# ShenhanQian/SpeechDrivesTemplates

Measured on AMD Instinct MI355X. Metric: training clips/sec (64-frame, 137-kpt) voice2pose_sdt_bp, higher is better.
Workload: dtype f32 (Conv2d forward / input gradient: each fp32 operand split exactly into three bf16 numbers, six bf16 MFMA products per fp32 product, fp32 accumulation -- products exact to 2^-23; everything else fp32 arithmetic)

## Files before the change

__graft_entry__.py:

```python
import os
import subprocess
import sys

REPO = os.path.dirname(os.path.abspath(__file__))
CSRC = os.path.join(REPO, "speechdrivestemplates_amd", "csrc")
LIBDIR = os.path.join(REPO, "speechdrivestemplates_amd", "lib")
LIB = os.path.join(LIBDIR, "libsdt_hip.so")
SOURCES = ["conv.hip", "convsk.hip", "convbf.hip", "norm.hip", "misc.hip", "l0.hip", "chain1d.hip", "render.hip", "speaker_stats.hip",
           "code_pca.hip", "code_axes.hip", "code_clusters.hip", "fgd.hip", "jpeg.hip", "gif.hip", "clip_builder.hip", "optim_guard.hip",
           "tensor_hist.hip", "reg_loss.hip", "bone_loss.hip", "clip_metrics.hip", "long_demo.hip", "sync_metrics.hip", "augment.hip", "speech_gate.hip",
           "pose_augment.hip", "motion_dist.hip", "code_fit.hip"]
HIPCC = os.environ.get("HIPCC", "/opt/rocm/bin/hipcc")
FLAGS = ["--offload-arch=gfx950", "-O3", "-std=c++17", "-fPIC", "-munsafe-fp-atomics", "-Wno-unused-result", "-Wno-unused-value"]


def _stale(out, deps):
    if not os.path.exists(out):
        return True
    t = os.path.getmtime(out)
    return any(os.path.getmtime(d) > t for d in deps)


TUNING_LIB = os.path.join(LIBDIR, "libsdt_hip_tuning.so")


def _headers():
# ... 111 lines not shown
```

include/sdt_hip.h:

```cpp
#ifndef SDT_HIP_H
#define SDT_HIP_H

#include <stdint.h>

#ifdef __cplusplus
extern "C" {
#endif

#define SDT_MAX_TAPS 20

enum sdt_status { SDT_OK = 0, SDT_ERR_ARG = -1, SDT_ERR_LAUNCH = -2, SDT_ERR_UNSUPPORTED = -3 };
enum sdt_dtype { SDT_F32 = 0, SDT_BF16 = 1 };

const char* sdt_last_error(void);
int sdt_abi_version(void);

typedef struct sdt_conv_geom {
    int32_t B, Hi, Wi, Cin;
    int32_t Ho, Wo;
    int32_t Hy, Wy, Cout;
    int32_t sy, sx;
    int32_t osy, osx, ooy, oox;
    int32_t ntaps, Tw;
    int32_t dy[SDT_MAX_TAPS], dx[SDT_MAX_TAPS], wt[SDT_MAX_TAPS];
// ... 54 lines not shown
int64_t sdt_convsk_dw_plan_bytes_t(const sdt_conv_geom* g, int dtype);
int sdt_convsk_dw_plan_build_t(const sdt_conv_geom* g, int dtype, void* out, int64_t out_bytes);
int sdt_convsk_dw_bf16(const void* x, const void* dy, float* dw, const void* plan_host, const void* plan_dev, void* workspace,
                       int64_t xbytes, int64_t ybytes, void* stream);
int sdt_conv_dw_f32(const float* x, const float* dy, float* dw, const sdt_conv_geom* g, void* stream);
int64_t sdt_conv_dw_workspace_bytes(const sdt_conv_geom* g);
int sdt_conv_dw_det_f32(const float* x, const float* dy, float* dw, const sdt_conv_geom* g, void* workspace, int64_t workspace_bytes,
                        void* stream);
int sdt_conv_taps_variant(const sdt_conv_geom* g);
int sdt_conv1d_small_used(const sdt_conv_geom* geoms, int ncls, int splitk);
int sdt_conv_dw_variant(const sdt_conv_geom* g);
int sdt_weight_transpose_f32(const float* w, float* wt, int cout, int taps, int cin, void* stream);
enum { SDT_MATH_F32 = 0, SDT_MATH_BF16 = 1, SDT_MATH_BF16X3 = 3, SDT_MATH_BF16X6 = 6 };
int sdt_set_conv_math(int mode);
int sdt_get_conv_math(void);


int64_t sdt_conv_dw_group_plan_bytes(int n);
int sdt_conv_dw_group_plan(const sdt_conv_geom* const* geoms, int n, void* plan_out, int64_t* workspace_bytes);
int sdt_conv_dw_group_f32(const void* const* x, const void* const* dy, void* const* dw, int n, const void* plan_host, const void* plan_dev,
                          void* workspace, void* stream);
typedef struct sdt_wt_desc {
    const float* w;
    float* wt;
    void* w16;
    void* wt16;
    int32_t cout, taps, cin, tile_begin;
    int32_t planes;
    int32_t reserved;
} sdt_wt_desc;
// ... 21 lines not shown

int sdt_l0_block_fwd_f32(const float* mel, const float* w, float* z, double* mom, float* mean, float* rstd,
                         const float* gamma, const float* beta, float* running_mean, float* running_var,
                         int64_t* num_batches_tracked, int B, int H, int W, int groups, float eps, float momentum,
                         float slope, void* stream);
int sdt_l0_block_bwd_f32(const float* dz, const float* mel, const float* w, const float* mean, const float* rstd,
                         const float* gamma, const float* beta, const double* mom, double* sums, float* dw, float* dgamma,
                         float* dbeta, int B, int H, int W, int groups, float slope, void* stream);
int sdt_l0_block_fwd_t(const float* mel, const float* w, void* z, int z_dtype, double* mom, float* mean, float* rstd,
                       const float* gamma, const float* beta, float* running_mean, float* running_var,
                       int64_t* num_batches_tracked, int B, int H, int W, int groups, float eps, float momentum,
                       float slope, void* stream);
int sdt_l0_block_bwd_t(const void* dz, int dz_dtype, const float* mel, const float* w, const float* mean, const float* rstd,
                       const float* gamma, const float* beta, const double* mom, double* sums, float* dw, float* dgamma,
                       float* dbeta, int B, int H, int W, int groups, float slope, void* stream);

int sdt_rownorm_fwd_f32(const float* y, float* z, float* mean, float* rstd, int64_t rows, int C,
                        float eps, float slope, void* stream);
int sdt_rownorm_bwd_f32(const float* dz, const float* y, const float* mean, const float* rstd, float* dy,
                        int64_t rows, int C, float slope, void* stream);
int sdt_rownorm_slabs_fwd_f32(const float* partial, int nslab, float* y, float* z, float* mean, float* rstd,
                              int64_t rows, int C, float eps, float slope, void* stream);

int sdt_resize_concat_fwd_f32(const float* x, const float* table, const int64_t* idx, float* out,
                              int B, int H, int W, int C, int T, int D, void* stream);
int sdt_resize_concat_bwd_f32(const float* dout, const int64_t* idx, float* dx, float* dtable,
                              int B, int H, int W, int C, int T, int D, void* stream);

int sdt_upsample_add_fwd_f32(const float* prev, const float* skip, float* out, int B, int Ti, int To, int C, void* stream);
int sdt_upsample_add_bwd_f32(const float* dout, float* dprev, int B, int Ti, int To, int C, void* stream);
// ... 40 lines not shown
int sdt_code_kl_fwd_f32(const float* table, const int64_t* idx, int N, int B, int D, float lambda,
                        float* code_out, float* loss, int32_t* valid, void* stream);
int sdt_code_kl_bwd_f32(const float* code, const int32_t* valid, const float* gout, const int64_t* idx,
                        int N, int B, int D, float lambda, float* dtable, void* stream);

int sdt_final_metrics_f64(const float* pred, const float* gt, const double* mean, const double* std,
                          const double* scale, int hierarchical, int B, int T, int K,
                          double* final_pred, double* final_gt, double* work, double* metrics, void* stream);

int sdt_adam_step_f32(float* p, const float* g, float* m, float* v, int64_t n, const float* lr_dev, float beta1,
                      float beta2, float eps, float weight_decay, float grad_scale, void* state_dev, void* stream);

int sdt_stft_frames_f32(const float* audio, float* hops, int B, int L, int nhops, void* stream);
int sdt_mel_fb_f32(const float* spec, const float* fb, const int32_t* bin_lo, const int32_t* bin_hi, float* mel, int B, int F,
                   int nfreq, int nmel, void* stream);

int sdt_rows_scatter_add_f32(const float* src, const int64_t* idx, float* dst, int N, int B, int D, void* stream);

int sdt_time_diff_fwd_f32(const float* x, float* y, int B, int T, int C, void* stream);
int sdt_time_diff_bwd_f32(const float* dy, float* dx, int B, int T, int C, void* stream);

int sdt_clip_poses_prepare_f32(const float* raw, const int64_t* idx, const float* mean, const float* std, float* poses,
                               float* score, int N, int Tstore, int B, int T, int hierarchical, void* stream);
int sdt_rows_gather_f32(const float* src, const int64_t* idx, float* dst, int N, int B, int64_t n_cols, void* stream);

typedef struct sdt_render_instance {
    int64_t pose;
    double off_x, off_y;
    double scale;
    int32_t shift_x;
// ... 208 lines not shown
```

speechdrivestemplates_amd/_lib.py:

```python
import ctypes as C
import os

_HERE = os.path.dirname(os.path.abspath(__file__))
LIB_PATH = os.environ.get("SDT_HIP_LIB") or os.path.join(_HERE, "lib", "libsdt_hip.so")
MAX_TAPS = 20
ABI_VERSION = 5


class ConvGeom(C.Structure):
    _fields_ = [(n, C.c_int32) for n in
                ("B", "Hi", "Wi", "Cin", "Ho", "Wo", "Hy", "Wy", "Cout", "sy", "sx", "osy", "osx", "ooy", "oox",
                 "ntaps", "Tw")] + [("dy", C.c_int32 * MAX_TAPS), ("dx", C.c_int32 * MAX_TAPS), ("wt", C.c_int32 * MAX_TAPS)]


class NormBwd(C.Structure):
    _fields_ = [("y", C.c_void_p), ("mean", C.c_void_p), ("rstd", C.c_void_p), ("gamma", C.c_void_p), ("beta", C.c_void_p),
                ("sums", C.c_void_p), ("slope", C.c_float), ("groups", C.c_int32)]


class WtDesc(C.Structure):
    _fields_ = [("w", C.c_void_p), ("wt", C.c_void_p), ("w16", C.c_void_p), ("wt16", C.c_void_p), ("cout", C.c_int32), ("taps", C.c_int32),
                ("cin", C.c_int32), ("tile_begin", C.c_int32), ("planes", C.c_int32), ("reserved", C.c_int32)]


# ... 48 lines not shown
    "sdt_l1_loss_fwd_f32": [_p, _p, _i64, _f, _p, _p, _p],
    "sdt_l1_loss_bwd_f32": [_p, _p, _p, _i64, _f, _p, _p],
    "sdt_reg_loss_fwd_f32": [_p, _p, _p, _p, _i, _i, _i, C.c_double, C.c_double, _f, _p, _p, _p, _p, _p],
    "sdt_reg_loss_bwd_f32": [_p, _p, _p, _p, _p, _p, _p, _i, _i, _i, C.c_double, C.c_double, _f, _p, _p],
    "sdt_bone_loss_fwd_f32": [_p, _p, _p, _p, _p, _p, _p, _p, _i, _i, _i, _i, C.c_double, C.c_double, _f, C.c_double, _p, _p, _p, _p, _p],
    "sdt_bone_loss_bwd_f32": [_p, _p, _p, _p, _p, _p, _p, _p, _p, _p, _p, _p, _p, _p, _p, _i, _i, _i, _i, C.c_double, C.c_double, _f,
                              C.c_double, _p, _p],
    "sdt_mse_const_fwd_f32": [_p, _i64, _f, _f, _p, _p],
    "sdt_mse_const_bwd_f32": [_p, _p, _i64, _f, _f, _p, _p],
    "sdt_code_kl_fwd_f32": [_p, _p, _i, _i, _i, _f, _p, _p, _p, _p],
    "sdt_code_kl_bwd_f32": [_p, _p, _p, _p, _i, _i, _i, _f, _p, _p],
    "sdt_final_metrics_f64": [_p, _p, _p, _p, _p, _i, _i, _i, _i, _p, _p, _p, _p, _p],
    "sdt_adam_step_f32": [_p, _p, _p, _p, _i64, _p, _f, _f, _f, _f, _f, _p, _p],
    "sdt_stft_frames_f32": [_p, _p, _i, _i, _i, _p],
    "sdt_mel_fb_f32": [_p, _p, _p, _p, _p, _i, _i, _i, _i, _p],
    "sdt_rows_scatter_add_f32": [_p, _p, _p, _i, _i, _i, _p],
    "sdt_time_diff_fwd_f32": [_p, _p, _i, _i, _i, _p],
    "sdt_time_diff_bwd_f32": [_p, _p, _i, _i, _i, _p],
    "sdt_clip_poses_prepare_f32": [_p, _p, _p, _p, _p, _p, _i, _i, _i, _i, _i, _p],
    "sdt_rows_gather_f32": [_p, _p, _p, _i, _i, _i64, _p],
    "sdt_convsk_supported": [_G, _i],
    "sdt_convsk_grid": [],
    "sdt_convsk_set_wg_per_cu": [_i],
    "sdt_convsk_set_f32_split": [_i],
    "sdt_convsk_set_reserved_slots": [_i],
    "sdt_convsk_plan_build": [_G, _i, _i, _i, _p, _i64],
    "sdt_convsk_dw_supported": [_G],
    "sdt_convsk_dw_plan_build": [_G, _p, _i64],
    "sdt_convsk_dw_f32": [_p, _p, _p, _p, _p, _p, _i64, _i64, _p],
    "sdt_convsk_f32": [_p, _p, _p, _p, _p, _p, _p, C.c_uint, _p, C.POINTER(NormBwd), _i64, _i64, _i64, _p],
# ... 204 lines not shown
```

speechdrivestemplates_amd/core/pipelines/voice2pose.py:

```python
import logging
import os
from collections import OrderedDict

import torch
from torch import nn

from ... import dp, ops
from ...config import check_augment, check_bone_loss, check_clip_metrics, check_fit_code, check_pose_augment, check_reg_loss
from ...mel import MelSpectrogram
from ...optim import FlatAdam
from ..datasets.gesture_dataset import PoseTransforms
from ..networks import get_model
from .trainer import Trainer


class Voice2PoseModel(nn.Module):
    def __init__(self, cfg, state_dict=None, num_train_samples=None, rank=0, external_codes=None) -> None:
        super().__init__()
        self.cfg = cfg
        self.reg_opts = check_reg_loss(cfg)
        self._chan_w = {}
        self.bone_opts = check_bone_loss(cfg)
        self.bone_table = None
        if self.bone_opts is not None:
# ... 106 lines not shown
            assert not return_loss, 'WARNING: Do not set "DEMO.CODE_INDEX" in train or test mode!'
            assert 0 <= self.cfg.DEMO.CODE_INDEX < table.size(0)
            c = table[torch.full((n,), self.cfg.DEMO.CODE_INDEX, dtype=torch.long, device=dev)]
            if interpolation_coeff is not None:
                assert self.cfg.DEMO.CODE_INDEX_B < table.size(0)
                cb = table[torch.full((n,), self.cfg.DEMO.CODE_INDEX_B, dtype=torch.long, device=dev)]
                c = c * (1 - interpolation_coeff) + cb * interpolation_coeff
            return c
        rows = self.num_clips if self.pose_aug_opts is not None and self.num_clips is not None else table.size(0)
        return table[torch.randint(min(rows, table.size(0)), (n,), device=dev)]

    def forward(self, batch, dataset, return_loss=True, interpolation_coeff=None, condition_code=None):
        cfg = self.cfg
        g = cfg.VOICE2POSE.GENERATOR
        dev = self._device()
        audio = batch['audio'].to(dev, non_blocking=True)
        speaker = batch['speaker']
        clip_indices = batch['clip_index'].to(dev, non_blocking=True)
        num_frames = int(batch['num_frames'][0])
        poses_gt = batch['poses'].to(dev, non_blocking=True) if return_loss else None
        poses_score = None
        if self.training and return_loss and self.pose_aug_opts is not None:
            from ...pose_augment import batch_poses
            want_score = (self.reg_opts is not None and self.reg_opts[1] is not None) or \
                         (self.bone_opts is not None and self.bone_opts[3] is not None)
            poses_gt, poses_score, code_rows = batch_poses(self._pose_augmenter(dev), batch, dev, want_score)
        else:
            code_rows = clip_indices

        kl = kl_valid = None
        if g.CLIP_CODE.DIMENSION is not None:
# ... 5 lines not shown
                                                     return_loss)
                if return_loss:
                    ar = torch.arange(condition_code.shape[0], device=dev)
                    _, kl, kl_valid = ops.CodeGatherKLFn.apply(condition_code.detach().contiguous(), ar, g.LAMBDA_CLIP_KL, True)
        else:
            condition_code = None

        if self.training and self.aug_opts is not None:
            if 'aug_step' not in batch:
                raise KeyError("TRAIN.AUGMENT.ENABLE is set but the batch has no 'aug_step' (an int64 tensor of shape (1,) with the global "
                               "step; Voice2Pose.train_step adds it): the augmentation depends on (seed, step, clip)")
            aug, aug_step = self._augmenter(dev), batch['aug_step'].to(dev, non_blocking=True)
            aug_clips = clip_indices.long().reshape(-1)
            audio = aug.audio(audio.float(), aug_clips, aug_step)
            mel = aug.mel_masks(self.mel_transfm(audio), aug_clips, aug_step)
        else:
            mel = self.mel_transfm(audio)
        poses_pred = self.netG(mel, num_frames, condition_code)
        results = {'poses_pred_batch': poses_pred, 'condition_code': condition_code}
        if not return_loss:
            return results
        results['poses_gt_batch'] = poses_gt

        losses = {}
        if self.reg_opts is None:
            reg = ops.L1LossFn.apply(poses_pred, poses_gt, float(g.LAMBDA_REG))
            losses['G_reg_loss'] = reg
            g_loss = reg
        else:
            lam_vel, min_conf, _ = self.reg_opts
# ... 124 lines not shown
                    lo_b = optg.offsets[i0]

                    def _launch_block_range(grad, _optg=optg, _lo=lo_b, _hi=hi, _r=reducer):
                        _r.launch(_optg, _lo, _hi)
                        return None

                    hooks[blk] = _launch_block_range
                    hi = lo_b
                self.model.netG.audio_encoder.grad_bucket_hooks = hooks

    ENCODER_BUCKET_BLOCKS = (5, 3, 1)

    def forward_backward(self, batch, want_final=False):
        dev = self.model._device()
        self.apply_knobs()
        ops.begin_step(dev)
        losses, results = self.model(batch, self.train_dataset)
        stat = batch['speaker_stat']
        pred, gt = results['poses_pred_batch'].detach(), results['poses_gt_batch']
        mean, std = stat['mean'].to(dev, non_blocking=True), stat['std'].to(dev, non_blocking=True)
        scale = stat['scale_factor'].to(dev, non_blocking=True)
        side = ops.side_stream_scope(True)
        with side:
            side.uses(pred, gt, mean, std, scale)
            fin_p, fin_g, metrics = ops.final_metrics(pred, gt, mean, std, scale, bool(self.cfg.DATASET.HIERARCHICAL_POSE),
                                                      want_final)
        results['poses_pred_normalized'] = results['poses_pred_batch']
        if want_final:
            results['poses_pred_batch'], results['poses_gt_batch'] = fin_p, fin_g
        losses['L2_dist'], losses['lip_sync_error_n'] = metrics[0], metrics[1]
# ... 317 lines not shown
```

speechdrivestemplates_amd/csrc/conv.hip:

```cpp
#include <stdlib.h>

#include "common.h"

#define BK 32
#define LDP 36
#define SDT_OOB 0x80000000u

#define SDT_MAX_CLASSES 4
struct geom_pack {
    sdt_conv_geom g[SDT_MAX_CLASSES];
    int mrot;
};
struct norm_bwd_args {
    const float* y;
    const float* mean;
    const float* rstd;
    const float* gamma;
    const float* beta;
    double* sums;
    float slope;
    int groups;
};

#ifdef SDT_TUNING
// ... 1428 lines not shown
static geom_pack pack_of(const sdt_conv_geom* const* gs, int n) {
    geom_pack gp;
    for (int i = 0; i < SDT_MAX_CLASSES; ++i) gp.g[i] = *gs[i < n ? i : 0];
    gp.mrot = 0;
    return gp;
}

#define SMALL1D_NS 8
static bool g_small1d = true;
#ifdef SDT_TUNING
extern "C" int sdt_debug_set_small1d(int on) {
    g_small1d = on != 0;
    return SDT_OK;
}
#endif
static bool small1d_ok(bool vec4, const sdt_conv_geom* const* gs, int ncls, int splitk, const norm_bwd_args& nb) {
    if (!g_small1d || !vec4 || g_conv_math != SDT_MATH_F32 || nb.sums != nullptr) return false;
    for (int c = 0; c < ncls; ++c) {
        const sdt_conv_geom& g = *gs[c];
        if (g.Hi != 1 || g.Ho != 1 || g.Hy != 1 || g.Cin % BK != 0 || g.Cout % 64 != 0) return false;
        const int nsteps_all = g.ntaps * (g.Cin / BK);
        if (cdiv(nsteps_all, splitk) > SMALL1D_NS) return false;
        for (int t = 0; t < g.ntaps; ++t)
            if (g.dy[t] != 0) return false;
    }
    return true;
}

template <int BM, int BN>
static void launch_taps(bool vec4, const float* x, const float* w, const float* bias, float* y,
                        const sdt_conv_geom* const* gs, int ncls, int splitk, float* partial, const norm_bwd_args& nb, hipStream_t s) {
    const sdt_conv_geom& g = *gs[0];
    const size_t ysize = (size_t)g.B * g.Hy * g.Wy * g.Cout;
    int tiles = 0;
    for (int c = 0; c < ncls; ++c) tiles = std::max(tiles, cdiv(gs[c]->B * gs[c]->Ho * gs[c]->Wo, BM) * cdiv(gs[c]->Cout, BN));
    dim3 grid(tiles, ncls, splitk);
    geom_pack gp = pack_of(gs, ncls);
    if (vec4 && ncls == 1 && splitk == 1 && g.ntaps >= 9) {
        int dymin = g.dy[0], dymax = g.dy[0];
        for (int t = 1; t < g.ntaps; ++t) dymin = std::min(dymin, g.dy[t]), dymax = std::max(dymax, g.dy[t]);
        const int nnb = cdiv(g.Cout, BN), nmb = cdiv(g.B * g.Ho * g.Wo, BM);
        if (dymax - dymin + 1 > g.Hi && 32 % nnb == 0 && 32 / nnb >= 4) {
            const int S = 32 / nnb;
            const double per_image = (double)g.Ho * g.Wo / BM, per_cu = std::max(1.0, (double)nmb * nnb / 256.0);
            gp.mrot = (int)std::max(1l, lround(per_image / per_cu)) % S;
        }
    }
    if (vec4 && g_conv_math != SDT_MATH_F32 && ncls == 1 && nb.sums == nullptr) {
        switch (g_conv_math) {
            case SDT_MATH_BF16: hipLaunchKernelGGL((conv_taps_bf_kernel<1, BM, BN>), dim3(tiles, 1, splitk), dim3(256), 0, s, x, w, bias, y, g, splitk, partial, ysize); break;
            case SDT_MATH_BF16X3: hipLaunchKernelGGL((conv_taps_bf_kernel<3, BM, BN>), dim3(tiles, 1, splitk), dim3(256), 0, s, x, w, bias, y, g, splitk, partial, ysize); break;
            default: hipLaunchKernelGGL((conv_taps_bf_kernel<6, BM, BN>), dim3(tiles, 1, splitk), dim3(256), 0, s, x, w, bias, y, g, splitk, partial, ysize); break;
        }
        return;
    }
    if (small1d_ok(vec4, gs, ncls, splitk, nb) && BM == 64 && BN == 64) {
        hipLaunchKernelGGL((conv1d_small_kernel<SMALL1D_NS>), grid, dim3(256), 0, s, x, w, bias, y, gp, splitk, partial, ysize);
        return;
    }
#define SDT_TAPS(PRIO) hipLaunchKernelGGL((conv_taps_kernel<BM, BN, true, PRIO>), grid, dim3(256), 0, s, x, w, bias, y, gp, splitk, partial, ysize, (double*)nullptr, 0, nb)
    if (nb.sums != nullptr) {
        hipLaunchKernelGGL((conv_taps_kernel<BM, BN, true, 0, 2>), grid, dim3(256), 0, s, x, w, bias, y, gp, splitk, partial, ysize, (double*)nullptr, 0, nb);
        return;
    }
#ifdef SDT_TUNING
    static const int prio = getenv("SDT_CONV_PRIO") ? atoi(getenv("SDT_CONV_PRIO")) : 0;
    if (vec4 && prio == 1) SDT_TAPS(1);
    else if (vec4 && prio == 2) SDT_TAPS(2);
    else if (vec4 && prio == 3) SDT_TAPS(3);
    else if (vec4 && prio == 4) SDT_TAPS(4);
    else if (vec4 && prio == 5) SDT_TAPS(5);
// ... 34 lines not shown
static int taps_variant(const sdt_conv_geom* g, bool aligned) {
    const int vec4 = ((g->Cin % BK == 0) && aligned) ? 1 : 0;
    const int64_t M = (int64_t)g->B * g->Ho * g->Wo;
#ifdef SDT_TUNING
    static const int forced = getenv("SDT_CONV_TILE") ? atoi(getenv("SDT_CONV_TILE")) : 0;
    if (forced == 64064 || forced == 64128 || forced == 128064 || forced == 128128) return forced * 10 + vec4;
#endif
    return 64064 * 10 + vec4;
}
extern "C" int sdt_conv_taps_variant(const sdt_conv_geom* g) { return g ? taps_variant(g, true) : SDT_ERR_ARG; }
extern "C" int sdt_conv1d_small_used(const sdt_conv_geom* geoms, int ncls, int splitk) {
    if (!geoms || ncls < 1 || ncls > SDT_MAX_CLASSES || splitk < 1) return SDT_ERR_ARG;
    const sdt_conv_geom* gs[SDT_MAX_CLASSES];
    for (int c = 0; c < ncls; ++c) gs[c] = geoms + c;
    const int var = taps_variant(gs[0], true);
    return (var / 10 == 64064 && small1d_ok(var % 10, gs, ncls, splitk, kNoNormBwd)) ? 1 : 0;
}

extern "C" int sdt_conv_taps_splitk_hint(const sdt_conv_geom* g) {
    if (!g) return SDT_ERR_ARG;
    const int var = taps_variant(g, true);
    const int bm = var / 10 / 1000, bn = var / 10 % 1000;
    const int64_t tiles = cdiv64((int64_t)g->B * g->Ho * g->Wo, bm) * cdiv(g->Cout, bn);
    const bool one_d = g->Hi == 1 && g->Ho == 1;
    if (tiles >= (one_d ? 768 : 192)) return 1;
    const int nsteps = (var % 10) ? g->ntaps * cdiv(g->Cin, BK) : cdiv(g->ntaps * g->Cin, BK);
    int k = (int)std::min<int64_t>(std::min<int64_t>(cdiv64(tiles >= 192 ? 1024 : 512, tiles), nsteps / 4), 16);
    return std::max(k, 1);
}

static int taps_dispatch(const float* x, const float* w, const float* bias, float* y, const sdt_conv_geom* const* gs, int ncls,
                         int splitk, float* partial, const norm_bwd_args& nb, void* stream) {
    const int var = taps_variant(gs[0], (((uintptr_t)x | (uintptr_t)w) % 16) == 0);
    const bool vec4 = var % 10;
    hipStream_t s = (hipStream_t)stream;
    switch (var / 10) {
#ifdef SDT_TUNING
        case 128064: launch_taps<128, 64>(vec4, x, w, bias, y, gs, ncls, splitk, partial, nb, s); break;
        case 64128: launch_taps<64, 128>(vec4, x, w, bias, y, gs, ncls, splitk, partial, nb, s); break;
        case 128128: launch_taps<128, 128>(vec4, x, w, bias, y, gs, ncls, splitk, partial, nb, s); break;
#endif
        default: launch_taps<64, 64>(vec4, x, w, bias, y, gs, ncls, splitk, partial, nb, s); break;
    }
    SDT_LAUNCH_CHECK();
    return SDT_OK;
}

extern "C" int sdt_conv_taps_splitk_f32(const float* x, const float* w, const float* bias, float* y,
                                        const sdt_conv_geom* g, int splitk, float* partial, void* stream) {
    int rc = check_geom(g);
    if (rc) return rc;
    SDT_CHECK_ARG(x && w && y, "null pointer");
    SDT_CHECK_ARG(splitk >= 1 && splitk <= 64 && (splitk == 1 || partial != nullptr), "bad split-K arguments");
    return taps_dispatch(x, w, bias, y, &g, 1, splitk, partial, kNoNormBwd, stream);
}

extern "C" int sdt_conv_taps_multi_f32(const float* x, const float* w, float* y, const sdt_conv_geom* geoms, int ncls, int splitk,
                                       float* partial, const sdt_norm_bwd* nbw, void* stream) {
    SDT_CHECK_ARG(geoms && ncls >= 1 && ncls <= SDT_MAX_CLASSES, "1..4 geometries per launch");
    const sdt_conv_geom* gs[SDT_MAX_CLASSES];
    for (int c = 0; c < ncls; ++c) {
        gs[c] = geoms + c;
        int rc = check_geom(gs[c]);
        if (rc) return rc;
        SDT_CHECK_ARG(gs[c]->B == gs[0]->B && gs[c]->Hi == gs[0]->Hi && gs[c]->Wi == gs[0]->Wi && gs[c]->Cin == gs[0]->Cin &&
                          gs[c]->Hy == gs[0]->Hy && gs[c]->Wy == gs[0]->Wy && gs[c]->Cout == gs[0]->Cout && gs[c]->Tw == gs[0]->Tw,
                      "the classes of one launch must share the X, W and Y tensors");
    }
    SDT_CHECK_ARG(x && w && y, "null pointer");
    SDT_CHECK_ARG(splitk >= 1 && splitk <= 64 && (splitk == 1 || partial != nullptr), "bad split-K arguments");
    SDT_CHECK_ARG(g_conv_math == SDT_MATH_F32 || (ncls == 1 && nbw == nullptr), "multi-class / fused-statistics launches exist for fp32 math only");
    norm_bwd_args nb = kNoNormBwd;
    if (nbw != nullptr) {
        SDT_CHECK_ARG(nbw->y && nbw->mean && nbw->rstd && nbw->sums, "null pointer in sdt_norm_bwd");
        SDT_CHECK_ARG(splitk == 1 && (gs[0]->Cin % BK == 0), "fused backward statistics need an unsplit vector-path launch");
        SDT_CHECK_ARG(nbw->groups == 1 || nbw->groups == gs[0]->B, "groups must be 1 (BatchNorm) or B (InstanceNorm)");
        for (int c = 0; c < ncls; ++c)
            SDT_CHECK_ARG(nbw->groups == 1 ? (int64_t)gs[c]->B * gs[c]->Ho * gs[c]->Wo >= 64 : gs[c]->Ho * gs[c]->Wo >= 64,
                          "a group must span at least one 64-row tile");
        SDT_CHECK_ARG((int64_t)gs[0]->B * gs[0]->Hy * gs[0]->Wy * gs[0]->Cout * 4 < (1ll << 31) - 4, "output tensor too large for the fused backward statistics");
        nb = {(const float*)nbw->y, nbw->mean, nbw->rstd, nbw->gamma, nbw->beta, nbw->sums, nbw->slope, nbw->groups};
    }
    return taps_dispatch(x, w, nullptr, y, gs, ncls, splitk, partial, nb, stream);
}

extern "C" int sdt_conv_taps_stats_supported(const sdt_conv_geom* g, int rows_per_group) {
    if (!g || check_geom(g) || rows_per_group < 64) return 0;
    const int64_t M = (int64_t)g->B * g->Ho * g->Wo;
    return (g->Cin % BK == 0) && g_conv_math == SDT_MATH_F32 && M % rows_per_group == 0 &&
           sdt_conv_taps_splitk_hint(g) == 1 && g->osy == 1 && g->osx == 1 && g->ooy == 0 && g->oox == 0 && g->Hy == g->Ho &&
           g->Wy == g->Wo;
}
extern "C" int sdt_conv_taps_stats_f32(const float* x, const float* w, const float* bias, float* y, const sdt_conv_geom* g,
                                       double* stats, int rows_per_group, void* stream) {
    int rc = check_geom(g);
    if (rc) return rc;
    SDT_CHECK_ARG(x && w && y && stats, "null pointer");
    SDT_CHECK_ARG(sdt_conv_taps_stats_supported(g, rows_per_group), "geometry not supported by the fused-statistics epilogue");
// ... 11 lines not shown
        hipLaunchKernelGGL((conv_taps_kernel<64, 64, true, 14, 1>), grid, dim3(256), 0, (hipStream_t)stream, x, w, bias, y, gp, 1,
                           (float*)nullptr, ysize, stats, rows_per_group, kNoNormBwd);
    else
#endif
        hipLaunchKernelGGL((conv_taps_kernel<64, 64, true, 0, 1>), grid, dim3(256), 0, (hipStream_t)stream, x, w, bias, y, gp, 1,
                           (float*)nullptr, ysize, stats, rows_per_group, kNoNormBwd);
    SDT_LAUNCH_CHECK();
    return SDT_OK;
}

extern "C" int sdt_conv_taps_f32(const float* x, const float* w, const float* bias, float* y,
                                 const sdt_conv_geom* g, void* stream) {
    return sdt_conv_taps_splitk_f32(x, w, bias, y, g, 1, nullptr, stream);
}

extern "C" int sdt_splitk_reduce_f32(const float* partial, const float* bias, float* y, int64_t n, int cout, int splitk,
                                     void* stream) {
    SDT_CHECK_ARG(partial && y && n > 0 && cout > 0 && splitk >= 1, "bad argument");
    const unsigned grid = (unsigned)std::max<int64_t>(1, std::min<int64_t>(cdiv64(n, 256), 2048));
    hipLaunchKernelGGL(splitk_reduce_kernel, dim3(grid), dim3(256), 0, (hipStream_t)stream, partial, bias, y, (size_t)n, cout, splitk);
    SDT_LAUNCH_CHECK();
    return SDT_OK;
}

template <int BM, int BN>
static void dw_split(bool vec4, const sdt_conv_geom& g, int& nsplit, int& rows, int& coltiles, int& ntiles) {
    const int M = g.B * g.Ho * g.Wo;
    coltiles = vec4 ? g.ntaps * cdiv(g.Cin, BN) : cdiv(g.ntaps * g.Cin, BN);
    ntiles = cdiv(g.Cout, BM);
    const int tiles = coltiles * ntiles;
// ... 188 lines not shown
```

speechdrivestemplates_amd/csrc/l0.hip:

```cpp
#include "common.h"

#define L0_C 64
#define L0_T 9
#define L0_NMOM 54

__device__ __forceinline__ void l0_gather(const float* __restrict__ mel, int H, int W, int y, int x, float (&nb)[L0_T]) {
#pragma unroll
    for (int dy = -1; dy <= 1; ++dy)
#pragma unroll
        for (int dx = -1; dx <= 1; ++dx) {
            const int yy = y + dy, xx = x + dx;
            nb[(dy + 1) * 3 + (dx + 1)] = ((unsigned)yy < (unsigned)H && (unsigned)xx < (unsigned)W) ? mel[(size_t)yy * W + xx] : 0.f;
        }
}

struct L0Window {
    float nb[L0_T];
    const float* r0;
    const float* r1;
    const float* r2;
    int W;
    __device__ __forceinline__ float at(const float* r, int x) const { return (r != nullptr && (unsigned)x < (unsigned)W) ? r[x] : 0.f; }
    __device__ __forceinline__ void init(const float* img, int H, int W_, int y, int x) {
        W = W_;
// ... 320 lines not shown
    if (j == 0) {
        double x = 0.0, y = 0.0;
        for (int i = 0; i < 32; ++i) x += sA[i][t], y += sB[i][t];
        const double dw = groups == 1 ? term(0, x, y) : x;
        dW[c * L0_T + t] += (float)dw;
        if (t == 0 && groups == 1) {
            const double* sg = sums + (size_t)c * L0_NSUM;
            if (dgamma) dgamma[c] += (float)sg[1];
            if (dbeta) dbeta[c] += (float)sg[0];
        }
    }
}

static int l0_ppb(int HW) { return std::max(1024, std::min(4096, cdiv(HW, 8) / 256 * 256)); }

extern "C" int sdt_l0_block_fwd_t(const float* mel, const float* w, void* z, int z_dtype, double* mom, float* mean, float* rstd,
                                  const float* gamma, const float* beta, float* running_mean, float* running_var,
                                  int64_t* num_batches_tracked, int B, int H, int W, int groups, float eps, float momentum,
                                  float slope, void* stream) {
    SDT_CHECK_ARG(mel && w && z && mom && mean && rstd, "null pointer");
    SDT_CHECK_ARG(z_dtype == SDT_F32 || z_dtype == SDT_BF16, "unknown element type");
    SDT_CHECK_ARG(B > 0 && H > 0 && W > 0 && (groups == B || groups == 1), "bad dims (groups must be B or 1)");
    SDT_CHECK_ARG((int64_t)B * H * W * L0_C * 4 < (1ll << 40), "tensor too large");
    hipStream_t s = (hipStream_t)stream;
    const int HW = H * W, ppb = l0_ppb(HW);
    dim3 grid(cdiv(HW, ppb), B);
    if (HW <= L0_FEW)
        hipLaunchKernelGGL(l0_moments_kernel<true>, grid, dim3(256), 0, s, mel, mom, H, W, ppb);
    else
        hipLaunchKernelGGL(l0_moments_kernel<false>, grid, dim3(256), 0, s, mel, mom, H, W, ppb);
    const double n = groups == 1 ? (double)B * HW : (double)HW;
    hipLaunchKernelGGL(l0_finalize_kernel, dim3(cdiv(groups * L0_C, 64)), dim3(64), 0, s, mom, w, mean, rstd, running_mean,
                       running_var, num_batches_tracked, B, groups, n, eps, momentum);
    if (z_dtype == SDT_F32)
        hipLaunchKernelGGL(l0_fwd_kernel<float>, dim3(H, B), dim3(256), 0, s, mel, w, mean, rstd, gamma, beta, (float*)z, H, W, groups, slope);
    else
        hipLaunchKernelGGL(l0_fwd_kernel<__bf16>, dim3(H, B), dim3(256), 0, s, mel, w, mean, rstd, gamma, beta, (__bf16*)z, H, W, groups, slope);
    SDT_LAUNCH_CHECK();
    return SDT_OK;
}
extern "C" int sdt_l0_block_fwd_f32(const float* mel, const float* w, float* z, double* mom, float* mean, float* rstd,
                                    const float* gamma, const float* beta, float* running_mean, float* running_var,
                                    int64_t* num_batches_tracked, int B, int H, int W, int groups, float eps, float momentum,
                                    float slope, void* stream) {
    return sdt_l0_block_fwd_t(mel, w, z, SDT_F32, mom, mean, rstd, gamma, beta, running_mean, running_var, num_batches_tracked, B, H, W, groups, eps,
                              momentum, slope, stream);
}

extern "C" int sdt_l0_block_bwd_t(const void* dz, int dz_dtype, const float* mel, const float* w, const float* mean, const float* rstd,
                                  const float* gamma, const float* beta, const double* mom, double* sums, float* dw,
                                  float* dgamma, float* dbeta, int B, int H, int W, int groups, float slope, void* stream) {
    SDT_CHECK_ARG(dz && mel && w && mean && rstd && mom && sums && dw, "null pointer");
    SDT_CHECK_ARG(dz_dtype == SDT_F32 || dz_dtype == SDT_BF16, "unknown element type");
    SDT_CHECK_ARG(B > 0 && H > 0 && W > 0 && (groups == B || groups == 1), "bad dims (groups must be B or 1)");
// ... 24 lines not shown
```

speechdrivestemplates_amd/ops.py:

```python
import functools
import math
import os

import torch

from . import _lib
from ._lib import ConvGeom, check

LEAKY_SLOPE = 0.2
BN_EPS, BN_MOMENTUM = 1e-5, 0.1


def out_size(n, k, s, p):
    return (n + 2 * p - k) // s + 1


def _geom(**kw):
    g = ConvGeom()
    taps = kw.pop("taps")
    for k, v in kw.items():
        setattr(g, k, int(v))
    g.ntaps = len(taps)
    assert 0 < g.ntaps <= _lib.MAX_TAPS, "kernel has too many taps (%d)" % g.ntaps
    for i, (dy, dx, wt) in enumerate(taps):
# ... 1247 lines not shown
        check(lib.sdt_colnorm_bwd_t(_p(gz), _dt(gz), _p(y), _dt(y), _p(dy), _dt(dy), _p(sums), _p(mean), _p(rstd), _p(gamma), _p(beta), _p(dg), _p(db),
                                    ctx.groups, R, C, ctx.slope, int(ready), _stream()))
        return dy, None, None, None, None, None, None, None, None, None, None


class L0BlockFn(torch.autograd.Function):

    @staticmethod
    def forward(ctx, mel, w, gamma, beta, rmean, rvar, nbt, groups, slope, holder=None):
        _req_cuda(mel, w)
        lib = _lib.load()
        mel = mel.contiguous()
        B, H, W = mel.shape
        ws = weight_storage(w)
        z = torch.empty((B, H, W, 64), device=mel.device, dtype=torch.bfloat16 if STORAGE == "bf16" else torch.float32)
        mom = _ARENA.take(54 * B, mel.device)
        mean = torch.empty(groups * 64, device=mel.device, dtype=torch.float32)
        rstd = torch.empty_like(mean)
        check(lib.sdt_l0_block_fwd_t(_p(mel), _p(ws), _p(z), _dt(z), _p(mom), _p(mean), _p(rstd), _p(gamma), _p(beta), _p(rmean),
                                     _p(rvar), _p(nbt), B, H, W, groups, BN_EPS, BN_MOMENTUM, slope, _stream()))
        ctx.save_for_backward(mel, w, mean, rstd, gamma, beta, mom)
        ctx.groups, ctx.slope = groups, slope
        return z

    @staticmethod
    def backward(ctx, gz):
        mel, w, mean, rstd, gamma, beta, mom = ctx.saved_tensors
        lib = _lib.load()
        gz = gz.contiguous()
        B, H, W = mel.shape
        sums = _ARENA.take(11 * ctx.groups * 64, mel.device)
        gw = grad_buffer(w)
        if weight_storage(gw).data_ptr() != gw.data_ptr():
            raise RuntimeError("weight gradient is not in the (Cout,taps,Cin) kernel layout")
        dg = grad_buffer(gamma) if gamma is not None and gamma.requires_grad else None
# ... 583 lines not shown
    math = _CONV_MATH_NOW[0]
    if math != 0:
        check(lib.sdt_set_conv_math(0))
    try:
        check(lib.sdt_conv_taps_f32(_p(hops), _p(basis), None, _p(spec), g, st))
    finally:
        if math != 0:
            check(lib.sdt_set_conv_math(math))
    nmel = fb.shape[1]
    mel = torch.empty((B, nmel, F), device=audio.device, dtype=torch.float32)
    fb = fb.contiguous()
    check(lib.sdt_mel_fb_f32(_p(spec), _p(fb), _p(lo), _p(hi), _p(mel), B, F, N_FREQ, nmel, st))
    return mel


def adam_step(p, g, m, v, lr_dev, state_dev, beta1=0.9, beta2=0.999, eps=1e-8, weight_decay=0.0, grad_scale=1.0):
    _req_cuda(p, g, m, v, lr_dev, state_dev)
    check(_lib.load().sdt_adam_step_f32(_p(p), _p(g), _p(m), _p(v), p.numel(), _p(lr_dev), beta1, beta2, eps, weight_decay,
                                        grad_scale, _p(state_dev), _stream()))


GUARD_WORDS = 4


def grad_sumsq_partials():
    return int(_lib.load().sdt_grad_sumsq_partials())


def optim_guard_pass_elems(which):
    return int(_lib.load().sdt_optim_guard_pass_elems({'sumsq': 0, 'adam': 1}[which]))
# ... 69 lines not shown
```

Before: 5804.

## Run audio STFT/mel frontend on a side stream overlapping step setup

```diff
diff --git a/__graft_entry__.py b/__graft_entry__.py
--- a/__graft_entry__.py
+++ b/__graft_entry__.py
@@ -9,7 +9,7 @@
 SOURCES = ["conv.hip", "convsk.hip", "convbf.hip", "norm.hip", "misc.hip", "l0.hip", "chain1d.hip", "render.hip", "speaker_stats.hip",
            "code_pca.hip", "code_axes.hip", "code_clusters.hip", "fgd.hip", "jpeg.hip", "gif.hip", "clip_builder.hip", "optim_guard.hip",
            "tensor_hist.hip", "reg_loss.hip", "bone_loss.hip", "clip_metrics.hip", "long_demo.hip", "sync_metrics.hip", "augment.hip", "speech_gate.hip",
-           "pose_augment.hip", "motion_dist.hip", "code_fit.hip"]
+           "pose_augment.hip", "motion_dist.hip", "code_fit.hip", "frontend.hip"]
 HIPCC = os.environ.get("HIPCC", "/opt/rocm/bin/hipcc")
 FLAGS = ["--offload-arch=gfx950", "-O3", "-std=c++17", "-fPIC", "-munsafe-fp-atomics", "-Wno-unused-result", "-Wno-unused-value"]
 
diff --git a/include/sdt_hip.h b/include/sdt_hip.h
--- a/include/sdt_hip.h
+++ b/include/sdt_hip.h
@@ -92,6 +92,7 @@
 enum { SDT_MATH_F32 = 0, SDT_MATH_BF16 = 1, SDT_MATH_BF16X3 = 3, SDT_MATH_BF16X6 = 6 };
 int sdt_set_conv_math(int mode);
 int sdt_get_conv_math(void);
+int sdt_conv_taps_math_f32(const float* x, const float* w, const float* bias, float* y, const sdt_conv_geom* g, int math, void* stream);
 
 
 int64_t sdt_conv_dw_group_plan_bytes(int n);
@@ -143,6 +144,11 @@
 int sdt_l0_block_bwd_t(const void* dz, int dz_dtype, const float* mel, const float* w, const float* mean, const float* rstd,
                        const float* gamma, const float* beta, const double* mom, double* sums, float* dw, float* dgamma,
                        float* dbeta, int B, int H, int W, int groups, float slope, void* stream);
+int sdt_l0_moments_f32(const float* mel, double* mom, int B, int H, int W, void* stream);
+int sdt_l0_block_fwd_mom_t(const float* mel, const float* w, void* z, int z_dtype, double* mom, float* mean, float* rstd,
+                           const float* gamma, const float* beta, float* running_mean, float* running_var,
+                           int64_t* num_batches_tracked, int B, int H, int W, int groups, float eps, float momentum,
+                           float slope, int mom_ready, void* stream);
 
 int sdt_rownorm_fwd_f32(const float* y, float* z, float* mean, float* rstd, int64_t rows, int C,
                         float eps, float slope, void* stream);
@@ -213,6 +219,8 @@
 int sdt_stft_frames_f32(const float* audio, float* hops, int B, int L, int nhops, void* stream);
 int sdt_mel_fb_f32(const float* spec, const float* fb, const int32_t* bin_lo, const int32_t* bin_hi, float* mel, int B, int F,
                    int nfreq, int nmel, void* stream);
+int sdt_audio_frontend_f32(const float* audio, const float* basis, const float* fb, const int32_t* bin_lo, const int32_t* bin_hi,
+                           float* hops, float* spec, float* mel, double* mom, int B, int L, int nfreq, int nmel, void* stream);
 
 int sdt_rows_scatter_add_f32(const float* src, const int64_t* idx, float* dst, int N, int B, int D, void* stream);
 
diff --git a/speechdrivestemplates_amd/_lib.py b/speechdrivestemplates_amd/_lib.py
--- a/speechdrivestemplates_amd/_lib.py
+++ b/speechdrivestemplates_amd/_lib.py
@@ -86,6 +86,10 @@
     "sdt_adam_step_f32": [_p, _p, _p, _p, _i64, _p, _f, _f, _f, _f, _f, _p, _p],
     "sdt_stft_frames_f32": [_p, _p, _i, _i, _i, _p],
     "sdt_mel_fb_f32": [_p, _p, _p, _p, _p, _i, _i, _i, _i, _p],
+    "sdt_audio_frontend_f32": [_p, _p, _p, _p, _p, _p, _p, _p, _p, _i, _i, _i, _i, _p],
+    "sdt_conv_taps_math_f32": [_p, _p, _p, _p, _G, _i, _p],
+    "sdt_l0_moments_f32": [_p, _p, _i, _i, _i, _p],
+    "sdt_l0_block_fwd_mom_t": [_p, _p, _p, _i, _p, _p, _p, _p, _p, _p, _p, _p, _i, _i, _i, _i, _f, _f, _f, _i, _p],
     "sdt_rows_scatter_add_f32": [_p, _p, _p, _i, _i, _i, _p],
     "sdt_time_diff_fwd_f32": [_p, _p, _i, _i, _i, _p],
     "sdt_time_diff_bwd_f32": [_p, _p, _i, _i, _i, _p],
diff --git a/speechdrivestemplates_amd/core/pipelines/voice2pose.py b/speechdrivestemplates_amd/core/pipelines/voice2pose.py
--- a/speechdrivestemplates_amd/core/pipelines/voice2pose.py
+++ b/speechdrivestemplates_amd/core/pipelines/voice2pose.py
@@ -144,7 +144,10 @@
         cfg = self.cfg
         g = cfg.VOICE2POSE.GENERATOR
         dev = self._device()
-        audio = batch['audio'].to(dev, non_blocking=True)
+        pre, self.frontend = getattr(self, 'frontend', None), None
+        if pre is not None and (pre.source is not batch['audio'] or not self.training or self.aug_opts is not None):
+            pre = None
+        audio = pre.audio if pre is not None else batch['audio'].to(dev, non_blocking=True)
         speaker = batch['speaker']
         clip_indices = batch['clip_index'].to(dev, non_blocking=True)
         num_frames = int(batch['num_frames'][0])
@@ -180,6 +183,8 @@
             aug_clips = clip_indices.long().reshape(-1)
             audio = aug.audio(audio.float(), aug_clips, aug_step)
             mel = aug.mel_masks(self.mel_transfm(audio), aug_clips, aug_step)
+        elif pre is not None:
+            mel = ops.frontend_consume(pre)
         else:
             mel = self.mel_transfm(audio)
         poses_pred = self.netG(mel, num_frames, condition_code)
@@ -334,6 +339,19 @@
     def forward_backward(self, batch, want_final=False):
         dev = self.model._device()
         self.apply_knobs()
+        pre = None
+        if self.model.training and self.model.aug_opts is None and torch.is_tensor(batch.get('audio')):
+            mt = self.model.mel_transfm
+            pre = ops.frontend_enqueue(batch['audio'], mt._dft_basis(), mt.mel_scale.fb, mt._fb_bins(), dev)
+        try:
+            return self._forward_backward(batch, want_final, dev, pre)
+        finally:
+            self.model.frontend = None
+            if pre is not None:
+                ops.frontend_release(pre)
+
+    def _forward_backward(self, batch, want_final, dev, pre):
+        self.model.frontend = pre
         ops.begin_step(dev)
         losses, results = self.model(batch, self.train_dataset)
         stat = batch['speaker_stat']
diff --git a/speechdrivestemplates_amd/csrc/conv.hip b/speechdrivestemplates_amd/csrc/conv.hip
--- a/speechdrivestemplates_amd/csrc/conv.hip
+++ b/speechdrivestemplates_amd/csrc/conv.hip
@@ -1466,8 +1466,8 @@
     return SDT_OK;
 }
 #endif
-static bool small1d_ok(bool vec4, const sdt_conv_geom* const* gs, int ncls, int splitk, const norm_bwd_args& nb) {
-    if (!g_small1d || !vec4 || g_conv_math != SDT_MATH_F32 || nb.sums != nullptr) return false;
+static bool small1d_ok(bool vec4, const sdt_conv_geom* const* gs, int ncls, int splitk, const norm_bwd_args& nb, int math) {
+    if (!g_small1d || !vec4 || math != SDT_MATH_F32 || nb.sums != nullptr) return false;
     for (int c = 0; c < ncls; ++c) {
         const sdt_conv_geom& g = *gs[c];
         if (g.Hi != 1 || g.Ho != 1 || g.Hy != 1 || g.Cin % BK != 0 || g.Cout % 64 != 0) return false;
@@ -1481,7 +1481,7 @@
 
 template <int BM, int BN>
 static void launch_taps(bool vec4, const float* x, const float* w, const float* bias, float* y,
-                        const sdt_conv_geom* const* gs, int ncls, int splitk, float* partial, const norm_bwd_args& nb, hipStream_t s) {
+                        const sdt_conv_geom* const* gs, int ncls, int splitk, float* partial, const norm_bwd_args& nb, int math, hipStream_t s) {
     const sdt_conv_geom& g = *gs[0];
     const size_t ysize = (size_t)g.B * g.Hy * g.Wy * g.Cout;
     int tiles = 0;
@@ -1498,15 +1498,15 @@
             gp.mrot = (int)std::max(1l, lround(per_image / per_cu)) % S;
         }
     }
-    if (vec4 && g_conv_math != SDT_MATH_F32 && ncls == 1 && nb.sums == nullptr) {
-        switch (g_conv_math) {
+    if (vec4 && math != SDT_MATH_F32 && ncls == 1 && nb.sums == nullptr) {
+        switch (math) {
             case SDT_MATH_BF16: hipLaunchKernelGGL((conv_taps_bf_kernel<1, BM, BN>), dim3(tiles, 1, splitk), dim3(256), 0, s, x, w, bias, y, g, splitk, partial, ysize); break;
             case SDT_MATH_BF16X3: hipLaunchKernelGGL((conv_taps_bf_kernel<3, BM, BN>), dim3(tiles, 1, splitk), dim3(256), 0, s, x, w, bias, y, g, splitk, partial, ysize); break;
             default: hipLaunchKernelGGL((conv_taps_bf_kernel<6, BM, BN>), dim3(tiles, 1, splitk), dim3(256), 0, s, x, w, bias, y, g, splitk, partial, ysize); break;
         }
         return;
     }
-    if (small1d_ok(vec4, gs, ncls, splitk, nb) && BM == 64 && BN == 64) {
+    if (small1d_ok(vec4, gs, ncls, splitk, nb, math) && BM == 64 && BN == 64) {
         hipLaunchKernelGGL((conv1d_small_kernel<SMALL1D_NS>), grid, dim3(256), 0, s, x, w, bias, y, gp, splitk, partial, ysize);
         return;
     }
@@ -1571,7 +1571,7 @@
     const sdt_conv_geom* gs[SDT_MAX_CLASSES];
     for (int c = 0; c < ncls; ++c) gs[c] = geoms + c;
     const int var = taps_variant(gs[0], true);
-    return (var / 10 == 64064 && small1d_ok(var % 10, gs, ncls, splitk, kNoNormBwd)) ? 1 : 0;
+    return (var / 10 == 64064 && small1d_ok(var % 10, gs, ncls, splitk, kNoNormBwd, g_conv_math)) ? 1 : 0;
 }
 
 extern "C" int sdt_conv_taps_splitk_hint(const sdt_conv_geom* g) {
@@ -1587,17 +1587,17 @@
 }
 
 static int taps_dispatch(const float* x, const float* w, const float* bias, float* y, const sdt_conv_geom* const* gs, int ncls,
-                         int splitk, float* partial, const norm_bwd_args& nb, void* stream) {
+                         int splitk, float* partial, const norm_bwd_args& nb, int math, void* stream) {
     const int var = taps_variant(gs[0], (((uintptr_t)x | (uintptr_t)w) % 16) == 0);
     const bool vec4 = var % 10;
     hipStream_t s = (hipStream_t)stream;
     switch (var / 10) {
 #ifdef SDT_TUNING
-        case 128064: launch_taps<128, 64>(vec4, x, w, bias, y, gs, ncls, splitk, partial, nb, s); break;
-        case 64128: launch_taps<64, 128>(vec4, x, w, bias, y, gs, ncls, splitk, partial, nb, s); break;
-        case 128128: launch_taps<128, 128>(vec4, x, w, bias, y, gs, ncls, splitk, partial, nb, s); break;
+        case 128064: launch_taps<128, 64>(vec4, x, w, bias, y, gs, ncls, splitk, partial, nb, math, s); break;
+        case 64128: launch_taps<64, 128>(vec4, x, w, bias, y, gs, ncls, splitk, partial, nb, math, s); break;
+        case 128128: launch_taps<128, 128>(vec4, x, w, bias, y, gs, ncls, splitk, partial, nb, math, s); break;
 #endif
-        default: launch_taps<64, 64>(vec4, x, w, bias, y, gs, ncls, splitk, partial, nb, s); break;
+        default: launch_taps<64, 64>(vec4, x, w, bias, y, gs, ncls, splitk, partial, nb, math, s); break;
     }
     SDT_LAUNCH_CHECK();
     return SDT_OK;
@@ -1609,7 +1609,7 @@
     if (rc) return rc;
     SDT_CHECK_ARG(x && w && y, "null pointer");
     SDT_CHECK_ARG(splitk >= 1 && splitk <= 64 && (splitk == 1 || partial != nullptr), "bad split-K arguments");
-    return taps_dispatch(x, w, bias, y, &g, 1, splitk, partial, kNoNormBwd, stream);
+    return taps_dispatch(x, w, bias, y, &g, 1, splitk, partial, kNoNormBwd, g_conv_math, stream);
 }
 
 extern "C" int sdt_conv_taps_multi_f32(const float* x, const float* w, float* y, const sdt_conv_geom* geoms, int ncls, int splitk,
@@ -1638,7 +1638,7 @@
         SDT_CHECK_ARG((int64_t)gs[0]->B * gs[0]->Hy * gs[0]->Wy * gs[0]->Cout * 4 < (1ll << 31) - 4, "output tensor too large for the fused backward statistics");
         nb = {(const float*)nbw->y, nbw->mean, nbw->rstd, nbw->gamma, nbw->beta, nbw->sums, nbw->slope, nbw->groups};
     }
-    return taps_dispatch(x, w, nullptr, y, gs, ncls, splitk, partial, nb, stream);
+    return taps_dispatch(x, w, nullptr, y, gs, ncls, splitk, partial, nb, g_conv_math, stream);
 }
 
 extern "C" int sdt_conv_taps_stats_supported(const sdt_conv_geom* g, int rows_per_group) {
@@ -1680,6 +1680,15 @@
     return sdt_conv_taps_splitk_f32(x, w, bias, y, g, 1, nullptr, stream);
 }
 
+extern "C" int sdt_conv_taps_math_f32(const float* x, const float* w, const float* bias, float* y, const sdt_conv_geom* g, int math,
+                                      void* stream) {
+    int rc = check_geom(g);
+    if (rc) return rc;
+    SDT_CHECK_ARG(x && w && y, "null pointer");
+    SDT_CHECK_ARG(math == SDT_MATH_F32 || math == SDT_MATH_BF16 || math == SDT_MATH_BF16X3 || math == SDT_MATH_BF16X6, "unknown math mode");
+    return taps_dispatch(x, w, bias, y, &g, 1, 1, nullptr, kNoNormBwd, math, stream);
+}
+
 extern "C" int sdt_splitk_reduce_f32(const float* partial, const float* bias, float* y, int64_t n, int cout, int splitk,
                                      void* stream) {
     SDT_CHECK_ARG(partial && y && n > 0 && cout > 0 && splitk >= 1, "bad argument");
diff --git a/speechdrivestemplates_amd/csrc/frontend.hip b/speechdrivestemplates_amd/csrc/frontend.hip
--- /dev/null
+++ b/speechdrivestemplates_amd/csrc/frontend.hip
@@ -0,0 +1,30 @@
+#include "common.h"
+
+#define FE_HOP 160
+
+extern "C" int sdt_audio_frontend_f32(const float* audio, const float* basis, const float* fb, const int32_t* bin_lo, const int32_t* bin_hi,
+                                      float* hops, float* spec, float* mel, double* mom, int B, int L, int nfreq, int nmel, void* stream) {
+    SDT_CHECK_ARG(audio && basis && fb && bin_lo && bin_hi && hops && spec && mel, "null pointer");
+    SDT_CHECK_ARG(B > 0 && L > 256 && nfreq > 0 && nmel > 0, "bad dims (L must exceed the 256-sample reflect pad)");
+    const int F = 1 + L / FE_HOP, nh = F + 2;
+    sdt_conv_geom g = {};
+    g.B = B, g.Hi = 1, g.Wi = nh, g.Cin = FE_HOP;
+    g.Ho = 1, g.Wo = F;
+    g.Hy = 1, g.Wy = F, g.Cout = 2 * nfreq;
+    g.sy = g.sx = g.osy = g.osx = 1;
+    g.ooy = g.oox = 0;
+    g.ntaps = g.Tw = 3;
+    for (int t = 0; t < 3; ++t) g.dy[t] = 0, g.dx[t] = t, g.wt[t] = t;
+    if (mom != nullptr && hipMemsetAsync(mom, 0, (size_t)B * 54 * sizeof(double), (hipStream_t)stream) != hipSuccess) {
+        sdt_set_error("%s: clearing the moment record failed", __func__);
+        return SDT_ERR_LAUNCH;
+    }
+    int rc = sdt_stft_frames_f32(audio, hops, B, L, nh, stream);
+    if (rc) return rc;
+    rc = sdt_conv_taps_math_f32(hops, basis, nullptr, spec, &g, SDT_MATH_F32, stream);
+    if (rc) return rc;
+    rc = sdt_mel_fb_f32(spec, fb, bin_lo, bin_hi, mel, B, F, nfreq, nmel, stream);
+    if (rc) return rc;
+    if (mom != nullptr) rc = sdt_l0_moments_f32(mel, mom, B, nmel, F, stream);
+    return rc;
+}
diff --git a/speechdrivestemplates_amd/csrc/l0.hip b/speechdrivestemplates_amd/csrc/l0.hip
--- a/speechdrivestemplates_amd/csrc/l0.hip
+++ b/speechdrivestemplates_amd/csrc/l0.hip
@@ -358,14 +358,9 @@
 
 static int l0_ppb(int HW) { return std::max(1024, std::min(4096, cdiv(HW, 8) / 256 * 256)); }
 
-extern "C" int sdt_l0_block_fwd_t(const float* mel, const float* w, void* z, int z_dtype, double* mom, float* mean, float* rstd,
-                                  const float* gamma, const float* beta, float* running_mean, float* running_var,
-                                  int64_t* num_batches_tracked, int B, int H, int W, int groups, float eps, float momentum,
-                                  float slope, void* stream) {
-    SDT_CHECK_ARG(mel && w && z && mom && mean && rstd, "null pointer");
-    SDT_CHECK_ARG(z_dtype == SDT_F32 || z_dtype == SDT_BF16, "unknown element type");
-    SDT_CHECK_ARG(B > 0 && H > 0 && W > 0 && (groups == B || groups == 1), "bad dims (groups must be B or 1)");
-    SDT_CHECK_ARG((int64_t)B * H * W * L0_C * 4 < (1ll << 40), "tensor too large");
+extern "C" int sdt_l0_moments_f32(const float* mel, double* mom, int B, int H, int W, void* stream) {
+    SDT_CHECK_ARG(mel && mom, "null pointer");
+    SDT_CHECK_ARG(B > 0 && H > 0 && W > 0 && (int64_t)H * W < (1ll << 31), "bad dims");
     hipStream_t s = (hipStream_t)stream;
     const int HW = H * W, ppb = l0_ppb(HW);
     dim3 grid(cdiv(HW, ppb), B);
@@ -373,6 +368,24 @@
         hipLaunchKernelGGL(l0_moments_kernel<true>, grid, dim3(256), 0, s, mel, mom, H, W, ppb);
     else
         hipLaunchKernelGGL(l0_moments_kernel<false>, grid, dim3(256), 0, s, mel, mom, H, W, ppb);
+    SDT_LAUNCH_CHECK();
+    return SDT_OK;
+}
+
+extern "C" int sdt_l0_block_fwd_mom_t(const float* mel, const float* w, void* z, int z_dtype, double* mom, float* mean, float* rstd,
+                                      const float* gamma, const float* beta, float* running_mean, float* running_var,
+                                      int64_t* num_batches_tracked, int B, int H, int W, int groups, float eps, float momentum,
+                                      float slope, int mom_ready, void* stream) {
+    SDT_CHECK_ARG(mel && w && z && mom && mean && rstd, "null pointer");
+    SDT_CHECK_ARG(z_dtype == SDT_F32 || z_dtype == SDT_BF16, "unknown element type");
+    SDT_CHECK_ARG(B > 0 && H > 0 && W > 0 && (groups == B || groups == 1), "bad dims (groups must be B or 1)");
+    SDT_CHECK_ARG((int64_t)B * H * W * L0_C * 4 < (1ll << 40), "tensor too large");
+    hipStream_t s = (hipStream_t)stream;
+    const int HW = H * W;
+    if (!mom_ready) {
+        int rc = sdt_l0_moments_f32(mel, mom, B, H, W, stream);
+        if (rc) return rc;
+    }
     const double n = groups == 1 ? (double)B * HW : (double)HW;
     hipLaunchKernelGGL(l0_finalize_kernel, dim3(cdiv(groups * L0_C, 64)), dim3(64), 0, s, mom, w, mean, rstd, running_mean,
                        running_var, num_batches_tracked, B, groups, n, eps, momentum);
@@ -382,6 +395,13 @@
         hipLaunchKernelGGL(l0_fwd_kernel<__bf16>, dim3(H, B), dim3(256), 0, s, mel, w, mean, rstd, gamma, beta, (__bf16*)z, H, W, groups, slope);
     SDT_LAUNCH_CHECK();
     return SDT_OK;
+}
+extern "C" int sdt_l0_block_fwd_t(const float* mel, const float* w, void* z, int z_dtype, double* mom, float* mean, float* rstd,
+                                  const float* gamma, const float* beta, float* running_mean, float* running_var,
+                                  int64_t* num_batches_tracked, int B, int H, int W, int groups, float eps, float momentum,
+                                  float slope, void* stream) {
+    return sdt_l0_block_fwd_mom_t(mel, w, z, z_dtype, mom, mean, rstd, gamma, beta, running_mean, running_var, num_batches_tracked, B, H, W, groups,
+                                  eps, momentum, slope, 0, stream);
 }
 extern "C" int sdt_l0_block_fwd_f32(const float* mel, const float* w, float* z, double* mom, float* mean, float* rstd,
                                     const float* gamma, const float* beta, float* running_mean, float* running_var,
diff --git a/speechdrivestemplates_amd/ops.py b/speechdrivestemplates_amd/ops.py
--- a/speechdrivestemplates_amd/ops.py
+++ b/speechdrivestemplates_amd/ops.py
@@ -1285,11 +1285,14 @@
         B, H, W = mel.shape
         ws = weight_storage(w)
         z = torch.empty((B, H, W, 64), device=mel.device, dtype=torch.bfloat16 if STORAGE == "bf16" else torch.float32)
-        mom = _ARENA.take(54 * B, mel.device)
+        mom = _frontend_moments(mel)
+        ready = mom is not None
+        if not ready:
+            mom = _ARENA.take(54 * B, mel.device)
         mean = torch.empty(groups * 64, device=mel.device, dtype=torch.float32)
         rstd = torch.empty_like(mean)
-        check(lib.sdt_l0_block_fwd_t(_p(mel), _p(ws), _p(z), _dt(z), _p(mom), _p(mean), _p(rstd), _p(gamma), _p(beta), _p(rmean),
-                                     _p(rvar), _p(nbt), B, H, W, groups, BN_EPS, BN_MOMENTUM, slope, _stream()))
+        check(lib.sdt_l0_block_fwd_mom_t(_p(mel), _p(ws), _p(z), _dt(z), _p(mom), _p(mean), _p(rstd), _p(gamma), _p(beta), _p(rmean),
+                                         _p(rvar), _p(nbt), B, H, W, groups, BN_EPS, BN_MOMENTUM, slope, int(ready), _stream()))
         ctx.save_for_backward(mel, w, mean, rstd, gamma, beta, mom)
         ctx.groups, ctx.slope = groups, slope
         return z
@@ -1903,6 +1906,132 @@
     return mel
 
 
+OVERLAP_FRONTEND = True
+_FE_STREAMS = {}
+_FE_SETS = {}
+_FE_TURN = {}
+_FE_MOMENTS = {}
+_FE_CONSTS = {}
+_AUDIO_SEEN = {}
+
+
+class _FrontEndSet:
+    def __init__(self, dev, B, L, nmel):
+        F = 1 + L // HOP
+        self.hops = torch.empty((B, F + 2, HOP), device=dev, dtype=torch.float32)
+        self.spec = torch.empty((B, F, 2 * N_FREQ), device=dev, dtype=torch.float32)
+        self.mel = torch.empty((B, nmel, F), device=dev, dtype=torch.float32)
+        self.mom = torch.empty(54 * B, device=dev, dtype=torch.float64)
+        self.done = torch.cuda.Event()
+        self.free = torch.cuda.Event()
+        self.read = False
+
+
+class FrontEnd:
+
+    def __init__(self, source, audio, bufs):
+        self.source, self.audio, self.bufs = source, audio, bufs
+
+
+def frontend_overlap_ok():
+    return bool(OVERLAP_FRONTEND and OVERLAP_AUX and torch.cuda.is_available() and not torch.cuda.is_current_stream_capturing())
+
+
+def _audio_ready_event(t):
+    import weakref
+    key = (t.data_ptr(), tuple(t.shape))
+    ent = _AUDIO_SEEN.get(key)
+    if ent is not None and ent[0]() is t and ent[1] == t._version:
+        return ent[2]
+    if len(_AUDIO_SEEN) >= 64:
+        for k in [k for k, v in _AUDIO_SEEN.items() if v[0]() is None]:
+            del _AUDIO_SEEN[k]
+        if len(_AUDIO_SEEN) >= 64:
+            _AUDIO_SEEN.clear()
+    ev = torch.cuda.Event()
+    ev.record()
+    _AUDIO_SEEN[key] = (weakref.ref(t), t._version, ev)
+    return ev
+
+
+def frontend_enqueue(source, basis, fb, bins, dev):
+    if not frontend_overlap_ok() or source.dim() != 2 or source.dtype != torch.float32 or source.shape[1] <= 256:
+        return None
+    dev = torch.device(dev)
+    di = dev.index if dev.index is not None else torch.cuda.current_device()
+    if source.is_cuda and (source.device.index != di or not source.is_contiguous()):
+        return None
+    _req_cuda(basis, fb)
+    lib = _lib.load()
+    fe = _FE_STREAMS.get(di)
+    if fe is None:
+        fe = _FE_STREAMS[di] = torch.cuda.Stream(device=di)
+    B, L = source.shape
+    nmel = fb.shape[1]
+    turn = _FE_TURN[di] = _FE_TURN.get(di, 0) ^ 1
+    key = (di, B, L, nmel, turn)
+    bufs = _FE_SETS.get(key)
+    if bufs is None:
+        if len(_FE_SETS) >= 8:
+            _FE_SETS.clear()
+        bufs = _FE_SETS[key] = _FrontEndSet(dev, B, L, nmel)
+    lo, hi = bins
+    consts = [(t, t._version) for t in (basis, fb, lo, hi)]
+    seen = _FE_CONSTS.get(di)
+    if seen is None or any(a is not b or va != vb for (a, va), (b, vb) in zip(seen, consts)):
+        fe.wait_stream(torch.cuda.current_stream())
+        _FE_CONSTS[di] = consts
+    if source.is_cuda:
+        fe.wait_event(_audio_ready_event(source))
+        audio = source
+    if bufs.read:
+        fe.wait_event(bufs.free)
+    with torch.cuda.stream(fe):
+        if not source.is_cuda:
+            audio = source.to(dev, non_blocking=True).contiguous()
+        check(lib.sdt_audio_frontend_f32(_p(audio), _p(basis), _p(fb.contiguous()), _p(lo), _p(hi), _p(bufs.hops), _p(bufs.spec), _p(bufs.mel),
+                                         _p(bufs.mom), B, L, N_FREQ, nmel, _stream()))
+        bufs.done.record()
+    if source.is_cuda:
+        audio.record_stream(fe)
+    return FrontEnd(source, audio, bufs)
+
+
+def frontend_consume(pre):
+    torch.cuda.current_stream().wait_event(pre.bufs.done)
+    mel = pre.bufs.mel
+    _FE_MOMENTS[(mel.device.index, mel.data_ptr())] = (pre.bufs.mom, tuple(mel.shape))
+    return mel
+
+
+def frontend_release(pre):
+    _FE_MOMENTS.pop((pre.bufs.mel.device.index, pre.bufs.mel.data_ptr()), None)
+    pre.bufs.free.record()
+    pre.bufs.read = True
+
+
+def _frontend_moments(mel):
+    ent = _FE_MOMENTS.pop((mel.device.index, mel.data_ptr()), None) if _FE_MOMENTS else None
+    return ent[0] if ent is not None and ent[1] == tuple(mel.shape) else None
+
+
+def audio_frontend(audio, basis, fb, bins=None, moments=True):
+    _req_cuda(audio, basis, fb)
+    lo, hi = bins if bins is not None else fb_bin_ranges(fb)
+    audio = audio.contiguous()
+    B, L = audio.shape
+    F = 1 + L // HOP
+    nmel = fb.shape[1]
+    dev = audio.device
+    hops = torch.empty((B, F + 2, HOP), device=dev, dtype=torch.float32)
+    spec = torch.empty((B, F, 2 * N_FREQ), device=dev, dtype=torch.float32)
+    mel = torch.empty((B, nmel, F), device=dev, dtype=torch.float32)
+    mom = torch.empty((B, 54), device=dev, dtype=torch.float64) if moments else None
+    check(_lib.load().sdt_audio_frontend_f32(_p(audio), _p(basis), _p(fb.contiguous()), _p(lo), _p(hi), _p(hops), _p(spec), _p(mel), _p(mom),
+                                             B, L, N_FREQ, nmel, _stream()))
+    return mel, mom
+
+
 def adam_step(p, g, m, v, lr_dev, state_dev, beta1=0.9, beta2=0.999, eps=1e-8, weight_decay=0.0, grad_scale=1.0):
     _req_cuda(p, g, m, v, lr_dev, state_dev)
     check(_lib.load().sdt_adam_step_f32(_p(p), _p(g), _p(m), _p(v), p.numel(), _p(lr_dev), beta1, beta2, eps, weight_decay,
```

After: 5800. About the same (-0.1%).
